# vwxyzjn/cleanrl

Hardware: NVIDIA H100
Metric: env steps/sec (SPS) PPO Breakout num_envs=1024 (higher is better)
Workload: dtype bf16

## Files before the change

### cleanrl_b200/csrc/net_tc.cu

```cuda
#include <cuda.h>
#include <algorithm>
#include "tc_base.cuh"
#include "tc_conv_win.cuh"
#include "tc_conv1_u8.cuh"
#include "tc_gemm_tma.cuh"
#include "tc_wgrad_win.cuh"
#include "tc_reduce.cuh"
#include "tc_aux.cuh"
#include "tc_heads.cuh"
#include "tc_heads_wide.cuh"
#include "tc_lstm.cuh"

namespace b200rl {

struct NatureLayout {
    int A;
    int64_t c1w, c1b, c2w, c2b, c3w, c3b, fcw, fcb, hw, hb, total;
    int64_t w1f, w2f, w2dg, w3f, w3dg, wfcf, wfcdg, w1l, w1sc, packed_total;
    bool wide; int G; int64_t whf, whdg, hbp;
    int64_t wih, whh, bih, bhh, whhp;
    explicit NatureLayout(int A_) : A(A_), wih(-1), whh(-1), bih(-1), bhh(-1), whhp(-1) {
        int64_t o = 0;
        c1w = o; o += 32 * 4 * 8 * 8;  c1b = o; o += 32;
        c2w = o; o += 64 * 32 * 4 * 4; c2b = o; o += 64;
        c3w = o; o += 64 * 64 * 3 * 3; c3b = o; o += 64;
        fcw = o; o += 512 * 3136;      fcb = o; o += 512;
        hw = o;  o += (int64_t)(A + 1) * 512;
        hb = o;  o += A + 1;
        total = o;
        int64_t q = 0;
        w1f = q; q += 32 * 256;
        w2f = q; q += 64 * 512;
        w2dg = q; q += 4 * 32 * 256;
        w3f = q; q += 64 * 576;
        w3dg = q; q += 64 * 576;
        wfcf = q; q += 512 * 3136;
        wfcdg = q; q += 3136 * 512;
        w1l = q; q += 64 * 256 / 2;
        w1sc = q; q += 64 * 2;
        wide = A + 1 > kMaxHeads;
        G = wide ? (int)ceil_div(A + 1, kWideHeadPad) * kWideHeadPad : 0;
        whf = whdg = hbp = 0;
        if (wide) {
            whf = q; q += (int64_t)G * 512;
            whdg = q; q += (int64_t)G * 512;
            hbp = q; q += (int64_t)G * 2;
        }
        packed_total = q;
    }
    struct Lstm {};
    NatureLayout(int A_, Lstm) : A(A_) {
        int64_t o = 0;
        c1w = o; o += 32 * 8 * 8;      c1b = o; o += 32;
        c2w = o; o += 64 * 32 * 4 * 4; c2b = o; o += 64;
        c3w = o; o += 64 * 64 * 3 * 3; c3b = o; o += 64;
        fcw = o; o += 512 * 3136;      fcb = o; o += 512;
        wih = o; o += 512 * 512;       whh = o; o += 512 * 128;
        bih = o; o += 512;             bhh = o; o += 512;
        hw = o;  o += (int64_t)(A + 1) * 128;
        hb = o;  o += A + 1;
        total = o;
        int64_t q = 0;
        w1f = q; q += 32 * 64;
        w2f = q; q += 64 * 512;
        w2dg = q; q += 4 * 32 * 256;
        w3f = q; q += 64 * 576;
        w3dg = q; q += 64 * 576;
        wfcf = q; q += 512 * 3136;
        wfcdg = q; q += 3136 * 512;
        w1l = w1sc = -1;
        wide = true; G = 512;
        whf = q; q += 512 * 512;
        whdg = q; q += 512 * 512;
        hbp = q; q += 512 * 2;
        whhp = q; q += 512 * 128;
        packed_total = q;
    }
};

struct NatureActs {
    int64_t x0, act1, act2, act3, hid, dhid, dact3a, dact3b, dact2a, dact2b, dact1, m1, m2, m3, m4, total;
    explicit NatureActs(int64_t n, bool with_x0 = true) {
        int64_t o = 0;
        x0 = o; if (with_x0) o += n * 28224;
        act1 = o; o += n * 12800;
        act2 = o; o += n * 5184;
        act3 = o; o += n * 3136;
        hid = o;  o += n * 512;
        dhid = o; o += n * 512;
        dact3a = o; o += n * 5184;
        dact3b = o; o += n * 7744;
        dact2a = o; o += n * 6400;
        dact2b = o; o += n * 7744;
        dact1 = o; o += n * 14112;
        auto pad8 = [](int64_t v) { return (v + 7) & ~int64_t(7); };
        m1 = o; o += pad8(n * 100 * 4 * 2);
        m2 = o; o += pad8(n * 81 * 2 * 2);
        m3 = o; o += pad8(n * 49 * 2 * 2);
        m4 = o; o += pad8(n * 16 * 2);
        total = o;
    }
};

static void gemm_rowmajor(KGemmParams& p, const bf16* x, int64_t n, int nchunks) {
    memset(&p, 0, sizeof(p));
    p.scale = 1.f;
    p.A = x; p.M = n; p.nchunks = nchunks;
}


static void win_defaults(WinParams& p) { memset(&p, 0, sizeof(p)); p.scale = 1.f; }
static int round8(int v) { return (v + 7) & ~7; }
static void win_conv1(WinParams& p, const bf16* x0, const int64_t* rows, int64_t n) {
    p.A = x0; p.rows = rows; p.n = (int)n; p.G = 441; p.Wp = 21; p.M = n * 441;
    p.tpi_shift = 2;
    p.n_images = rows ? (int64_t)1 << 24 : n;
    p.ntaps = 4; p.shift[0] = 0; p.shift[1] = 1; p.shift[2] = 21; p.shift[3] = 22; p.WR = round8(128 + 22);
}
static void win_conv2(WinParams& p, const bf16* act1, int64_t n) {
    p.A = act1; p.n = (int)n; p.G = 100; p.Wp = 10; p.M = n * 100;
    p.ntaps = 4; p.shift[0] = 0; p.shift[1] = 1; p.shift[2] = 10; p.shift[3] = 11; p.WR = round8(128 + 11);
}
static void win_conv3(WinParams& p, const bf16* act2, int64_t n) {
    p.A = act2; p.n = (int)n; p.G = 81; p.Wp = 9; p.M = n * 81;
    p.ntaps = 9; for (int ky = 0; ky < 3; ++ky) for (int kx = 0; kx < 3; ++kx) p.shift[ky * 3 + kx] = ky * 9 + kx;
    p.WR = round8(128 + 20);
}
static void wgw_defaults(WGradWinParams& w) { memset(&w, 0, sizeof(w)); }

static const int kC1Ctas = 264, kC2Ctas = 132, kC3Ctas = 132;
static WPlan conv1_wgrad_plan(int64_t n, bool u8) {
    return u8 ? wgrad_plan(n * 512, kC2Ctas, 512) : wgrad_plan(n * 512, kC1Ctas, 128);
}
static WPlan conv2_wgrad_plan(int64_t n) { return wgrad_plan(n * 100, kC2Ctas, 128); }
static WPlan conv3_wgrad_plan(int64_t n) { return wgrad_plan(n * 81, kC3Ctas, 128); }

static size_t wgrad_win_bytes(int splits, int nslots) { return (size_t)splits * nslots * 64 * 64 * sizeof(float); }
static size_t wgrad_win_bias_bytes(int splits) { return (size_t)splits * 64 * sizeof(float); }
static int launch_wgrad_win(const WGradWinParams& p, int ctas, cudaStream_t s, const char* what) {
    const size_t smem = (size_t)kWgradWinStages * ((size_t)p.WRX * 128 * p.cpr + 128 * 128) + 4096 + 1024;
    static SmemAttrCache attr;
    if (int rc0 = attr.ensure(tc_wgrad_win, smem, what)) return rc0;
    CUtensorMap tmX, tmY;
    memset(&tmX, 0, sizeof(tmX)); memset(&tmY, 0, sizeof(tmY));
    const int use_tma = p.tpi_shift ? 0 : 1;
    if (p.rows_per_cta % 128 != 0) return fail(B200RL_ERR_INVALID_ARGUMENT, "%s: rows per CTA must be a multiple of 128", what);
    if (ctas < 1 || (int64_t)(ctas - 1) * p.rows_per_cta >= p.M)
        return fail(B200RL_ERR_INVALID_ARGUMENT, "%s: every row split must own at least one row", what);
    int rc;
    if (use_tma) {
        if (p.rows || p.ldy != 64 || p.ncolsY != 64)
            return fail(B200RL_ERR_INVALID_ARGUMENT, "%s: linear-grid mode needs contiguous rows and 64-channel dY", what);
        if ((rc = make_tmap_2d(&tmX, p.X, p.M, (int64_t)p.cpr * 64, p.WRX, what))) return rc;
        if ((rc = make_tmap_2d(&tmY, p.Y, p.M, 64, 128, what))) return rc;
    } else {
        if ((128 << p.tpi_shift) < p.G) return fail(B200RL_ERR_INVALID_ARGUMENT, "%s: steps per image too small", what);
        if ((rc = make_tmap_3d(&tmX, p.X, p.n_images, p.G, (int64_t)p.cpr * 64, p.WRX, what))) return rc;
    }
    const dim3 grid((unsigned)ceil_div(p.nslots / 2, kWgradWinTilesPerCta), ctas);
    tc_wgrad_win<<<grid, kWgradWinThreads, smem, s>>>(tmX, tmY, p, use_tma);
    return check_launch(what);
}

}

using namespace b200rl;

namespace b200rl {
static bool head_ok(int A) { return A >= 1 && A < kMaxWideHeads; }
static size_t wide_dhead_bytes(int64_t n, const NatureLayout& L) { return ((size_t)n * L.G * 2 + 255) & ~(size_t)255; }
static size_t wide_small_bytes(int64_t n, const NatureLayout& L, int A1) {
    return wide_dhead_bytes(n, L) + colsum_f32_ws(n, A1);
}

static int trunk_fwd(const NatureLayout& L, const NatureActs& Q, const float* params, const bf16* P, bf16* act, int64_t n,
                     cudaStream_t s) {
    int rc;
    KGemmParams p;
    WinParams wp;
    win_defaults(wp); win_conv2(wp, act + Q.act1, n);
    wp.Bw = P + L.w2f; wp.N = 64; wp.vH = 9; wp.vW = 9; wp.out_mode = WOUT_DENSE; wp.out = act + Q.act2;
    wp.bias = params + L.c2b; wp.relu = 1; wp.mask_out = reinterpret_cast<uint32_t*>(act + Q.m2);
    { ProfScope ps(s, "conv2_fwd", 2.0 * n * 81 * 64 * 512, (double)n * ((12800 + 5184) * 2 + 648));
      if ((rc = launch_conv_win_t<128, 2, 2, 4>(wp, s, "naturecnn/conv2"))) return rc; }
    win_defaults(wp); win_conv3(wp, act + Q.act2, n);
    wp.Bw = P + L.w3f; wp.N = 64; wp.vH = 7; wp.vW = 7; wp.out_mode = WOUT_DENSE; wp.out = act + Q.act3;
    wp.bias = params + L.c3b; wp.relu = 1; wp.mask_out = reinterpret_cast<uint32_t*>(act + Q.m3);
    { ProfScope ps(s, "conv3_fwd", 2.0 * n * 49 * 64 * 576, (double)n * ((5184 + 3136) * 2 + 392));
      if ((rc = launch_conv_win_t<128, 1, 4, 9>(wp, s, "naturecnn/conv3"))) return rc; }
    gemm_rowmajor(p, act + Q.act3, n, 49);
    p.Bw = P + L.wfcf; p.N = 512; p.out = act + Q.hid; p.ldo = 512; p.bias = params + L.fcb; p.relu = 1;
    p.mask_out = reinterpret_cast<uint32_t*>(act + Q.m4);
    { ProfScope ps(s, "fc_fwd", 2.0 * n * 512 * 3136, (double)n * (3136 + 512) * 2 + 512.0 * 3136 * 2);
      if (n <= 8192) { if ((rc = launch_gemm_tma<64, 6>(p, s, "naturecnn/fc"))) return rc; }
      else if ((rc = launch_gemm_tma<128, 4>(p, s, "naturecnn/fc"))) return rc; }
    return B200RL_OK;
}

static int trunk_bwd(const NatureLayout& L, const NatureActs& Q, const bf16* P, bf16* act, float* grads, int64_t n,
                     float* wsbig, float* wssmall, void* tail_ready_event, bool dact1_fused, cudaStream_t s) {
    int rc;
    KGemmParams p;
    {
        int splits;
        { ProfScope ps(s, "fc_wgrad", 2.0 * n * 512 * 3136, (double)n * (3136 + 512) * 2 + 512.0 * 3136 * 4);
          if ((splits = launch_wgrad_tma(act + Q.dhid, 512, act + Q.act3, 3136, n, wsbig, s, "naturecnn/fc_wgrad")) < 0) return splits; }
        { ProfScope ps(s, "wgrad_fold_bias", 0, 0);
          note_launches(1); tc_fold_fc<<<(unsigned)ceil_div((int64_t)512 * 3136, 256), 256, 0, s>>>(wsbig, splits, 512, 13 * 256, 512, 3136, 64, 49, 1.f, grads + L.fcw);
          if ((rc = colsum(act + Q.dhid, n, 512, 512, wssmall, grads + L.fcb, s))) return rc; }
        if (tail_ready_event) {
            cudaError_t e = cudaEventRecord(reinterpret_cast<cudaEvent_t>(tail_ready_event), s);
            if (e != cudaSuccess) return fail(B200RL_ERR_CUDA, "naturecnn_backward: cudaEventRecord: %s", cudaGetErrorString(e));
        }
        gemm_rowmajor(p, act + Q.dhid, n, 8);
        p.Bw = P + L.wfcdg; p.N = 3136; p.out = act + Q.dact3a; p.out2 = act + Q.dact3b; p.dual_dact3 = 1;
        p.ldo = 3136; p.mask_bits = reinterpret_cast<const uint32_t*>(act + Q.m3);
        { ProfScope ps(s, "fc_dgrad", 2.0 * n * 512 * 3136, (double)n * ((3136 + 512) * 2 + 392) + 512.0 * 3136 * 2);
          if ((rc = launch_gemm_tma<128, 4>(p, s, "naturecnn/fc_dgrad"))) return rc; }
    }
    WGradWinParams gw;
    WinParams wp;
    FoldWin fw;
    {
        wgw_defaults(gw);
        gw.X = act + Q.act2; gw.M = n * 81; gw.n = (int)n; gw.G = 81; gw.cpr = 1; gw.nslots = 10; gw.WRX = round8(128 + 20);
        for (int t = 0; t < 9; ++t) gw.shift[t] = (t / 3) * 9 + (t % 3);
        const int st[10] = {0, 1, 2, 3, 4, 5, 6, 7, 7, 8};
        for (int k = 0; k < 10; ++k) { gw.slot_tap[k] = st[k]; gw.slot_cc[k] = 0; }
        gw.Y = act + Q.dact3a; gw.ldy = 64; gw.ncolsY = 64;
        const WPlan pl = conv3_wgrad_plan(n);
        gw.rows_per_cta = pl.rows_per_cta; gw.ws = wsbig; gw.wsb = wssmall;
        { ProfScope ps(s, "conv3_wgrad", 2.0 * n * 49 * 64 * 576, (double)n * (5184 + 5184) * 2);
          if ((rc = launch_wgrad_win(gw, pl.splits, s, "naturecnn/conv3_wgrad"))) return rc; }
        memset(&fw, 0, sizeof(fw));
        fw.layer = 3; fw.S = pl.splits; fw.nslots = 10; fw.Cout = 64; fw.scale = 1.f; fw.bscale = 1.f;
        for (int k = 0; k < 10; ++k) { fw.slot_tap[k] = st[k]; fw.slot_skip[k] = (k == 8); }
        { ProfScope ps(s, "wgrad_fold_bias", 0, 0);
          fw.wsb = wssmall; fw.db = grads + L.c3b;
          tc_fold_win<<<(unsigned)ceil_div(640 * 64 + 64, 32), 256, 0, s>>>(wsbig, fw, grads + L.c3w);
          if ((rc = check_launch("naturecnn/conv3_fold"))) return rc; }
        win_defaults(wp);
        wp.A = act + Q.dact3b; wp.n = (int)n; wp.G = 121; wp.Wp = 11; wp.M = n * 121; wp.ntaps = 9;
        for (int ky = 0; ky < 3; ++ky) for (int kx = 0; kx < 3; ++kx) wp.shift[ky * 3 + kx] = (2 - ky) * 11 + (2 - kx);
        wp.WR = round8(128 + 24);
        wp.Bw = P + L.w3dg; wp.N = 64; wp.vH = 9; wp.vW = 9; wp.out_mode = WOUT_DACT2;
        wp.out = act + Q.dact2a; wp.out2 = act + Q.dact2b; wp.mask_bits = reinterpret_cast<const uint32_t*>(act + Q.m2);
        { ProfScope ps(s, "conv3_dgrad", 2.0 * n * 81 * 64 * 576, (double)n * ((7744 + 6400 + 7744) * 2 + 648));
          if ((rc = launch_conv_win_t<128, 1, 4, 9>(wp, s, "naturecnn/conv3_dgrad"))) return rc; }
    }
    {
        wgw_defaults(gw);
        gw.X = act + Q.act1; gw.M = n * 100; gw.n = (int)n; gw.G = 100; gw.cpr = 2; gw.nslots = 8; gw.WRX = round8(128 + 11);
        gw.shift[0] = 0; gw.shift[1] = 1; gw.shift[2] = 10; gw.shift[3] = 11;
        for (int k = 0; k < 8; ++k) { gw.slot_tap[k] = k >> 1; gw.slot_cc[k] = k & 1; }
        gw.Y = act + Q.dact2a; gw.ldy = 64; gw.ncolsY = 64;
        const WPlan pl = conv2_wgrad_plan(n);
        gw.rows_per_cta = pl.rows_per_cta; gw.ws = wsbig; gw.wsb = wssmall;
        { ProfScope ps(s, "conv2_wgrad", 2.0 * n * 81 * 64 * 512, (double)n * (12800 + 6400) * 2);
          if ((rc = launch_wgrad_win(gw, pl.splits, s, "naturecnn/conv2_wgrad"))) return rc; }
        memset(&fw, 0, sizeof(fw));
        fw.layer = 2; fw.S = pl.splits; fw.nslots = 8; fw.Cout = 64; fw.scale = 1.f; fw.bscale = 1.f;
        for (int k = 0; k < 8; ++k) { fw.slot_tap[k] = k >> 1; fw.slot_cc[k] = k & 1; }
        { ProfScope ps(s, "wgrad_fold_bias", 0, 0);
          fw.wsb = wssmall; fw.db = grads + L.c2b;
          tc_fold_win<<<(unsigned)ceil_div(512 * 64 + 64, 32), 256, 0, s>>>(wsbig, fw, grads + L.c2w);
          if ((rc = check_launch("naturecnn/conv2_fold"))) return rc; }
        if (dact1_fused) return B200RL_OK;
        win_defaults(wp);
        wp.A = act + Q.dact2b; wp.n = (int)n; wp.G = 121; wp.Wp = 11; wp.M = n * 121; wp.ntaps = 4;
        for (int a = 0; a < 2; ++a) for (int b = 0; b < 2; ++b) wp.shift[a * 2 + b] = (1 - a) * 11 + (1 - b);
        wp.WR = round8(128 + 12);
        wp.Bw = P + L.w2dg; wp.N = 128; wp.vH = 10; wp.vW = 10; wp.out_mode = WOUT_DACT1;
        wp.out = act + Q.dact1; wp.mask_bits = reinterpret_cast<const uint32_t*>(act + Q.m1);
        { ProfScope ps(s, "conv2_dgrad", 2.0 * n * 400 * 32 * 256, (double)n * ((7744 + 14112) * 2 + 1600));
          if ((rc = launch_conv_win<128, 1, 4, 4>(wp, s, "naturecnn/conv2_dgrad"))) return rc; }
    }
    return B200RL_OK;
}
static size_t trunk_big_bytes(int64_t n) {
    return std::max({wgrad_tma_bytes(n, 512, 3136), wgrad_win_bytes(conv3_wgrad_plan(n).splits, 10),
                     wgrad_win_bytes(conv2_wgrad_plan(n).splits, 8)});
}
static size_t trunk_small_bytes(int64_t n) {
    return std::max({colsum_ws(n, 512), wgrad_win_bias_bytes(conv3_wgrad_plan(n).splits),
                     wgrad_win_bias_bytes(conv2_wgrad_plan(n).splits)});
}

static int wide_head_fwd(const NatureLayout& L, const bf16* P, const bf16* hid, int64_t n, int A1, float* out, cudaStream_t s) {
    KGemmParams p;
    gemm_rowmajor(p, hid, n, 8);
    p.Bw = P + L.whf; p.N = L.G; p.bias = reinterpret_cast<const float*>(P + L.hbp);
    p.out_f32 = out; p.ldo = A1; p.ncols_f32 = A1;
    return launch_gemm_tma<128, 4>(p, s, "wide_heads");
}

static int wide_head_bwd(const NatureLayout& L, const bf16* P, const float* dhead, int64_t n, int A1, const bf16* hid, bf16* dhid,
                         const uint32_t* hid_bits, float* dW, float* db, float* wsbig, float* wssmall, cudaStream_t s) {
    int rc;
    KGemmParams p;
    bf16* dh16 = reinterpret_cast<bf16*>(wssmall);
    float* dbpart = reinterpret_cast<float*>(reinterpret_cast<char*>(wssmall) + wide_dhead_bytes(n, L));
    int cb = (int)ceil_div(n * L.G, 256); if (cb > num_sms() * 8) cb = num_sms() * 8;
    tc_head_dhead_bf16<<<cb, 256, 0, s>>>(dhead, n, A1, L.G, dh16);
    if ((rc = check_launch("wide_heads_dhead"))) return rc;
    if ((rc = colsum_f32(dhead, n, A1, dbpart, db, s))) return rc;
    const int splits = launch_wgrad_tma(dh16, L.G, hid, 512, n, wsbig, s, "wide_heads_wgrad");
    if (splits < 0) return splits;
    tc_fold_fc<<<(unsigned)ceil_div((int64_t)A1 * 512, 256), 256, 0, s>>>(wsbig, splits, L.G, 512, A1, 512, 512, 1, 1.f, dW);
    if ((rc = check_launch("wide_heads_wgrad"))) return rc;
    gemm_rowmajor(p, dh16, n, L.G / 64);
    p.Bw = P + L.whdg; p.N = 512; p.out = dhid; p.ldo = 512;
    p.mask_bits = hid_bits;
    if (n <= 8192) { if ((rc = launch_gemm_tma<64, 6>(p, s, "wide_heads_dgrad"))) return rc; }
// ... 391 lines not shown
```

### cleanrl_b200/csrc/tc_wgmma.cuh

```cuda
#pragma once
#include <cstdint>

namespace b200rl { namespace tc {

__device__ __forceinline__ void wgmma_fence() { asm volatile("wgmma.fence.sync.aligned;" ::: "memory"); }
__device__ __forceinline__ void wgmma_commit() { asm volatile("wgmma.commit_group.sync.aligned;" ::: "memory"); }
template <int N>
__device__ __forceinline__ void wgmma_wait() { asm volatile("wgmma.wait_group.sync.aligned %0;" ::"n"(N) : "memory"); }
template <class T, int R>
__device__ __forceinline__ void wgmma_fence_operands(T (&d)[R]) {
#pragma unroll
    for (int i = 0; i < R; ++i) asm volatile("" : "+r"(reinterpret_cast<uint32_t&>(d[i]))::"memory");
}

template <int N, int TA, int TB> struct WgmmaBf16;
template <int TA, int TB> struct WgmmaBf16<32, TA, TB> {
    __device__ __forceinline__ static void mma(float (&d)[16], uint64_t adesc, uint64_t bdesc, uint32_t accumulate) {
        asm volatile(
            "{\n\t.reg .pred p;\n\tsetp.ne.b32 p, %18, 0;\n\t"
            "wgmma.mma_async.sync.aligned.m64n32k16.f32.bf16.bf16 {"
            "%0, %1, %2, %3, %4, %5, %6, %7, %8, %9, %10, %11, %12, %13, %14, %15"
            "}, %16, %17, p, 1, 1, %19, %20;\n\t}\n"
            : "+f"(d[0]), "+f"(d[1]), "+f"(d[2]), "+f"(d[3]), "+f"(d[4]), "+f"(d[5]), "+f"(d[6]), "+f"(d[7]),
              "+f"(d[8]), "+f"(d[9]), "+f"(d[10]), "+f"(d[11]), "+f"(d[12]), "+f"(d[13]), "+f"(d[14]), "+f"(d[15])
            : "l"(adesc), "l"(bdesc), "r"(accumulate), "n"(TA), "n"(TB));
    }
};
template <int TA, int TB> struct WgmmaBf16<64, TA, TB> {
    __device__ __forceinline__ static void mma(float (&d)[32], uint64_t adesc, uint64_t bdesc, uint32_t accumulate) {
        asm volatile(
            "{\n\t.reg .pred p;\n\tsetp.ne.b32 p, %34, 0;\n\t"
            "wgmma.mma_async.sync.aligned.m64n64k16.f32.bf16.bf16 {"
            "%0, %1, %2, %3, %4, %5, %6, %7, %8, %9, %10, %11, %12, %13, %14, %15, "
            "%16, %17, %18, %19, %20, %21, %22, %23, %24, %25, %26, %27, %28, %29, %30, %31"
            "}, %32, %33, p, 1, 1, %35, %36;\n\t}\n"
            : "+f"(d[0]), "+f"(d[1]), "+f"(d[2]), "+f"(d[3]), "+f"(d[4]), "+f"(d[5]), "+f"(d[6]), "+f"(d[7]),
              "+f"(d[8]), "+f"(d[9]), "+f"(d[10]), "+f"(d[11]), "+f"(d[12]), "+f"(d[13]), "+f"(d[14]), "+f"(d[15]),
              "+f"(d[16]), "+f"(d[17]), "+f"(d[18]), "+f"(d[19]), "+f"(d[20]), "+f"(d[21]), "+f"(d[22]), "+f"(d[23]),
              "+f"(d[24]), "+f"(d[25]), "+f"(d[26]), "+f"(d[27]), "+f"(d[28]), "+f"(d[29]), "+f"(d[30]), "+f"(d[31])
            : "l"(adesc), "l"(bdesc), "r"(accumulate), "n"(TA), "n"(TB));
    }
};
template <int TA, int TB> struct WgmmaBf16<128, TA, TB> {
    __device__ __forceinline__ static void mma(float (&d)[64], uint64_t adesc, uint64_t bdesc, uint32_t accumulate) {
        asm volatile(
            "{\n\t.reg .pred p;\n\tsetp.ne.b32 p, %66, 0;\n\t"
            "wgmma.mma_async.sync.aligned.m64n128k16.f32.bf16.bf16 {"
            "%0, %1, %2, %3, %4, %5, %6, %7, %8, %9, %10, %11, %12, %13, %14, %15, "
            "%16, %17, %18, %19, %20, %21, %22, %23, %24, %25, %26, %27, %28, %29, %30, %31, "
            "%32, %33, %34, %35, %36, %37, %38, %39, %40, %41, %42, %43, %44, %45, %46, %47, "
            "%48, %49, %50, %51, %52, %53, %54, %55, %56, %57, %58, %59, %60, %61, %62, %63"
            "}, %64, %65, p, 1, 1, %67, %68;\n\t}\n"
            : "+f"(d[0]), "+f"(d[1]), "+f"(d[2]), "+f"(d[3]), "+f"(d[4]), "+f"(d[5]), "+f"(d[6]), "+f"(d[7]),
              "+f"(d[8]), "+f"(d[9]), "+f"(d[10]), "+f"(d[11]), "+f"(d[12]), "+f"(d[13]), "+f"(d[14]), "+f"(d[15]),
              "+f"(d[16]), "+f"(d[17]), "+f"(d[18]), "+f"(d[19]), "+f"(d[20]), "+f"(d[21]), "+f"(d[22]), "+f"(d[23]),
              "+f"(d[24]), "+f"(d[25]), "+f"(d[26]), "+f"(d[27]), "+f"(d[28]), "+f"(d[29]), "+f"(d[30]), "+f"(d[31]),
              "+f"(d[32]), "+f"(d[33]), "+f"(d[34]), "+f"(d[35]), "+f"(d[36]), "+f"(d[37]), "+f"(d[38]), "+f"(d[39]),
              "+f"(d[40]), "+f"(d[41]), "+f"(d[42]), "+f"(d[43]), "+f"(d[44]), "+f"(d[45]), "+f"(d[46]), "+f"(d[47]),
              "+f"(d[48]), "+f"(d[49]), "+f"(d[50]), "+f"(d[51]), "+f"(d[52]), "+f"(d[53]), "+f"(d[54]), "+f"(d[55]),
              "+f"(d[56]), "+f"(d[57]), "+f"(d[58]), "+f"(d[59]), "+f"(d[60]), "+f"(d[61]), "+f"(d[62]), "+f"(d[63])
            : "l"(adesc), "l"(bdesc), "r"(accumulate), "n"(TA), "n"(TB));
    }
};
template <int TA, int TB> struct WgmmaBf16<256, TA, TB> {
    __device__ __forceinline__ static void mma(float (&d)[128], uint64_t adesc, uint64_t bdesc, uint32_t accumulate) {
        asm volatile(
            "{\n\t.reg .pred p;\n\tsetp.ne.b32 p, %130, 0;\n\t"
            "wgmma.mma_async.sync.aligned.m64n256k16.f32.bf16.bf16 {"
            "%0, %1, %2, %3, %4, %5, %6, %7, %8, %9, %10, %11, %12, %13, %14, %15, "
            "%16, %17, %18, %19, %20, %21, %22, %23, %24, %25, %26, %27, %28, %29, %30, %31, "
            "%32, %33, %34, %35, %36, %37, %38, %39, %40, %41, %42, %43, %44, %45, %46, %47, "
            "%48, %49, %50, %51, %52, %53, %54, %55, %56, %57, %58, %59, %60, %61, %62, %63, "
            "%64, %65, %66, %67, %68, %69, %70, %71, %72, %73, %74, %75, %76, %77, %78, %79, "
            "%80, %81, %82, %83, %84, %85, %86, %87, %88, %89, %90, %91, %92, %93, %94, %95, "
            "%96, %97, %98, %99, %100, %101, %102, %103, %104, %105, %106, %107, %108, %109, %110, %111, "
            "%112, %113, %114, %115, %116, %117, %118, %119, %120, %121, %122, %123, %124, %125, %126, %127"
            "}, %128, %129, p, 1, 1, %131, %132;\n\t}\n"
            : "+f"(d[0]), "+f"(d[1]), "+f"(d[2]), "+f"(d[3]), "+f"(d[4]), "+f"(d[5]), "+f"(d[6]), "+f"(d[7]),
              "+f"(d[8]), "+f"(d[9]), "+f"(d[10]), "+f"(d[11]), "+f"(d[12]), "+f"(d[13]), "+f"(d[14]), "+f"(d[15]),
              "+f"(d[16]), "+f"(d[17]), "+f"(d[18]), "+f"(d[19]), "+f"(d[20]), "+f"(d[21]), "+f"(d[22]), "+f"(d[23]),
              "+f"(d[24]), "+f"(d[25]), "+f"(d[26]), "+f"(d[27]), "+f"(d[28]), "+f"(d[29]), "+f"(d[30]), "+f"(d[31]),
              "+f"(d[32]), "+f"(d[33]), "+f"(d[34]), "+f"(d[35]), "+f"(d[36]), "+f"(d[37]), "+f"(d[38]), "+f"(d[39]),
              "+f"(d[40]), "+f"(d[41]), "+f"(d[42]), "+f"(d[43]), "+f"(d[44]), "+f"(d[45]), "+f"(d[46]), "+f"(d[47]),
              "+f"(d[48]), "+f"(d[49]), "+f"(d[50]), "+f"(d[51]), "+f"(d[52]), "+f"(d[53]), "+f"(d[54]), "+f"(d[55]),
              "+f"(d[56]), "+f"(d[57]), "+f"(d[58]), "+f"(d[59]), "+f"(d[60]), "+f"(d[61]), "+f"(d[62]), "+f"(d[63]),
              "+f"(d[64]), "+f"(d[65]), "+f"(d[66]), "+f"(d[67]), "+f"(d[68]), "+f"(d[69]), "+f"(d[70]), "+f"(d[71]),
              "+f"(d[72]), "+f"(d[73]), "+f"(d[74]), "+f"(d[75]), "+f"(d[76]), "+f"(d[77]), "+f"(d[78]), "+f"(d[79]),
              "+f"(d[80]), "+f"(d[81]), "+f"(d[82]), "+f"(d[83]), "+f"(d[84]), "+f"(d[85]), "+f"(d[86]), "+f"(d[87]),
              "+f"(d[88]), "+f"(d[89]), "+f"(d[90]), "+f"(d[91]), "+f"(d[92]), "+f"(d[93]), "+f"(d[94]), "+f"(d[95]),
              "+f"(d[96]), "+f"(d[97]), "+f"(d[98]), "+f"(d[99]), "+f"(d[100]), "+f"(d[101]), "+f"(d[102]), "+f"(d[103]),
              "+f"(d[104]), "+f"(d[105]), "+f"(d[106]), "+f"(d[107]), "+f"(d[108]), "+f"(d[109]), "+f"(d[110]), "+f"(d[111]),
              "+f"(d[112]), "+f"(d[113]), "+f"(d[114]), "+f"(d[115]), "+f"(d[116]), "+f"(d[117]), "+f"(d[118]), "+f"(d[119]),
              "+f"(d[120]), "+f"(d[121]), "+f"(d[122]), "+f"(d[123]), "+f"(d[124]), "+f"(d[125]), "+f"(d[126]), "+f"(d[127])
            : "l"(adesc), "l"(bdesc), "r"(accumulate), "n"(TA), "n"(TB));
    }
};

__device__ __forceinline__ void wgmma_u8s8_n64(int (&d)[32], uint64_t adesc, uint64_t bdesc, uint32_t accumulate) {
    asm volatile(
        "{\n\t.reg .pred p;\n\tsetp.ne.b32 p, %34, 0;\n\t"
        "wgmma.mma_async.sync.aligned.m64n64k32.s32.u8.s8 {"
        "%0, %1, %2, %3, %4, %5, %6, %7, %8, %9, %10, %11, %12, %13, %14, %15, "
        "%16, %17, %18, %19, %20, %21, %22, %23, %24, %25, %26, %27, %28, %29, %30, %31"
        "}, %32, %33, p;\n\t}\n"
        : "+r"(d[0]), "+r"(d[1]), "+r"(d[2]), "+r"(d[3]), "+r"(d[4]), "+r"(d[5]), "+r"(d[6]), "+r"(d[7]),
          "+r"(d[8]), "+r"(d[9]), "+r"(d[10]), "+r"(d[11]), "+r"(d[12]), "+r"(d[13]), "+r"(d[14]), "+r"(d[15]),
          "+r"(d[16]), "+r"(d[17]), "+r"(d[18]), "+r"(d[19]), "+r"(d[20]), "+r"(d[21]), "+r"(d[22]), "+r"(d[23]),
          "+r"(d[24]), "+r"(d[25]), "+r"(d[26]), "+r"(d[27]), "+r"(d[28]), "+r"(d[29]), "+r"(d[30]), "+r"(d[31])
        : "l"(adesc), "l"(bdesc), "r"(accumulate));
}

__device__ __forceinline__ void wgmma_f16_rs_n64_tb(float (&d)[32], const uint32_t (&a)[4], uint64_t bdesc, uint32_t accumulate) {
    asm volatile(
        "{\n\t.reg .pred p;\n\tsetp.ne.b32 p, %37, 0;\n\t"
        "wgmma.mma_async.sync.aligned.m64n64k16.f32.f16.f16 {"
        "%0, %1, %2, %3, %4, %5, %6, %7, %8, %9, %10, %11, %12, %13, %14, %15, "
        "%16, %17, %18, %19, %20, %21, %22, %23, %24, %25, %26, %27, %28, %29, %30, %31"
        "}, {%32, %33, %34, %35}, %36, p, 1, 1, 1;\n\t}\n"
        : "+f"(d[0]), "+f"(d[1]), "+f"(d[2]), "+f"(d[3]), "+f"(d[4]), "+f"(d[5]), "+f"(d[6]), "+f"(d[7]),
          "+f"(d[8]), "+f"(d[9]), "+f"(d[10]), "+f"(d[11]), "+f"(d[12]), "+f"(d[13]), "+f"(d[14]), "+f"(d[15]),
          "+f"(d[16]), "+f"(d[17]), "+f"(d[18]), "+f"(d[19]), "+f"(d[20]), "+f"(d[21]), "+f"(d[22]), "+f"(d[23]),
          "+f"(d[24]), "+f"(d[25]), "+f"(d[26]), "+f"(d[27]), "+f"(d[28]), "+f"(d[29]), "+f"(d[30]), "+f"(d[31])
        : "r"(a[0]), "r"(a[1]), "r"(a[2]), "r"(a[3]), "l"(bdesc), "r"(accumulate));
}

}}
```

### cleanrl_b200/csrc/tc_wgrad_win.cuh

```cuda
#pragma once
#include "tc_base.cuh"

namespace b200rl {
using namespace tc;

constexpr int kWgradWinStages = 3;
struct WGradWinParams {
    const bf16* X; const int64_t* rows; int64_t M; int n, G;
    int tpi_shift;
    int64_t n_images;
    int cpr;
    int nslots;
    int slot_tap[16], slot_cc[16];
    int shift[16];
    int WRX;
    const bf16* Y; int ldy, ncolsY;
    int64_t rows_per_cta;
    float* ws;
    float* wsb;
};

constexpr int kWgradWinThreads = 512;
constexpr int kWgradWinTilesPerCta = 2;

template <int NT>
__device__ __forceinline__ void wgrad_win_mma(const WGradWinParams& p, uint8_t* smem, int stage_bytes, int XBYTES, int IMGX,
                                              uint64_t* full_bar, uint64_t* empty_bar, int nsteps, int t0, int w, int tid) {
    constexpr int R = 128, STAGES = kWgradWinStages, NY = 64;
    const int wt = tid & 127;
    uint32_t arel[NT];
#pragma unroll
    for (int tt = 0; tt < NT; ++tt) {
        const int slot = 2 * (t0 + tt) + w;
        arel[tt] = (uint32_t)(p.slot_cc[slot] * IMGX + p.shift[p.slot_tap[slot]] * 128);
    }
    float d[NT][NY / 2];
#pragma unroll
    for (int tt = 0; tt < NT; ++tt)
#pragma unroll
        for (int e = 0; e < NY / 2; ++e) d[tt][e] = 0.f;
    auto step = [&](int it) {
        const int s = it % STAGES;
        mbar_wait(&full_bar[s], (it / STAGES) & 1);
        wgmma_fence();
        const uint32_t xa = smem_u32(smem + (size_t)s * stage_bytes), ya = xa + XBYTES;
        const uint64_t yd = desc_mnmajor(ya, 0);
#pragma unroll
        for (int tt = 0; tt < NT; ++tt) {
            const uint64_t xd = desc_mnmajor(xa + arel[tt], 0);
#pragma unroll
            for (int kk = 0; kk < R / 16; ++kk)
                WgmmaBf16<NY, 1, 1>::mma(d[tt], xd + kk * 128, yd + kk * 128, (it | kk) != 0 ? 1u : 0u);
        }
        wgmma_commit();
    };
    for (int it = 0; it + 1 < nsteps; ++it) {
        step(it);
        wgmma_wait<1>();
        if (it > 0 && (tid & 31) == 0) mbar_arrive(&empty_bar[(it - 1) % STAGES]);
    }
    step(nsteps - 1);
    wgmma_wait<0>();
    const int row = ((wt >> 5) << 4) + ((wt & 31) >> 2), col = (wt & 3) * 2;
    float* wsb = p.ws + (int64_t)blockIdx.y * (p.nslots * 64) * NY;
#pragma unroll
    for (int tt = 0; tt < NT; ++tt) {
        wgmma_fence_operands(d[tt]);
        float* d0 = wsb + (int64_t)((2 * (t0 + tt) + w) * 64 + row) * NY + col;
#pragma unroll
        for (int j = 0; j < NY / 8; ++j) {
            *reinterpret_cast<float2*>(d0 + 8 * j) = make_float2(d[tt][4 * j], d[tt][4 * j + 1]);
            *reinterpret_cast<float2*>(d0 + 8 * NY + 8 * j) = make_float2(d[tt][4 * j + 2], d[tt][4 * j + 3]);
        }
    }
}

static __global__ void __launch_bounds__(kWgradWinThreads, 1) tc_wgrad_win(const __grid_constant__ CUtensorMap tmX, const __grid_constant__ CUtensorMap tmY,
                                                       const WGradWinParams p, int use_tma) {
    constexpr int R = 128, STAGES = kWgradWinStages, LOOKAHEAD = 1, NY = 64, TT = kWgradWinTilesPerCta;
    static_assert(TT == 2, "the wgmma warpgroups dispatch on 1 or 2 tiles per CTA");
    extern __shared__ uint8_t smem_raw[];
    __shared__ uint64_t full_bar[STAGES], empty_bar[STAGES];
    uint8_t* smem = reinterpret_cast<uint8_t*>((reinterpret_cast<uintptr_t>(smem_raw) + 1023) & ~uintptr_t(1023));
    const int tid = threadIdx.x, warp = tid >> 5;
    const int IMGX = p.WRX * 128;
    const int XBYTES = IMGX * p.cpr;
    const int stage_bytes = XBYTES + R * 128;
    const int xt = p.nslots / 2;
    const int t0 = blockIdx.x * TT;
    float* sRed = reinterpret_cast<float*>(smem + (size_t)STAGES * stage_bytes);
    if (tid == 0) {
        for (int s = 0; s < STAGES; ++s) { mbar_init(&full_bar[s], use_tma ? 1 : 5); mbar_init(&empty_bar[s], (use_tma ? 4 : 0) + 8); }
        fence_barrier_init();
        tma_prefetch_desc(&tmX);
        if (use_tma) tma_prefetch_desc(&tmY);
    }
    __syncthreads();
    const int64_t m_begin = (int64_t)blockIdx.y * p.rows_per_cta;
    int64_t m_end = m_begin + p.rows_per_cta;
    if (m_end > p.M) m_end = p.M;
    const int nsteps = m_end > m_begin ? (int)((m_end - m_begin + R - 1) / R) : 0;
    const int tmask = (1 << p.tpi_shift) - 1;
    const int64_t g0 = m_begin / R;

    if (warp == 4) {
        if ((tid & 31) == 0) {
            int z_next = 0;
            if (!use_tma && nsteps > 0) {
                const int64_t img = g0 >> p.tpi_shift;
                z_next = p.rows ? (int)__ldg(p.rows + (img < p.n ? img : 0)) : (int)img;
            }
            for (int it = 0; it < nsteps; ++it) {
                const int s = it % STAGES;
                const int z = z_next;
                if (!use_tma && it + 1 < nsteps) {
                    const int64_t img1 = (g0 + it + 1) >> p.tpi_shift;
                    z_next = p.rows ? (int)__ldg(p.rows + (img1 < p.n ? img1 : 0)) : (int)img1;
                }
                if (it >= STAGES) mbar_wait(&empty_bar[s], ((it / STAGES) - 1) & 1);
                const uint32_t dst = smem_u32(smem + (size_t)s * stage_bytes);
                if (use_tma) {
                    const int m0 = (int)(m_begin + (int64_t)it * R);
                    mbar_arrive_expect_tx(&full_bar[s], (uint32_t)stage_bytes);
                    for (int c = 0; c < p.cpr; ++c) tma_load_2d(dst + c * IMGX, &tmX, c * 64, m0, &full_bar[s]);
                    tma_load_2d(dst + XBYTES, &tmY, 0, m0, &full_bar[s]);
                } else {
                    const int t_in = (int)((g0 + it) & tmask);
                    mbar_arrive_expect_tx(&full_bar[s], (uint32_t)XBYTES);
                    for (int c = 0; c < p.cpr; ++c) tma_load_3d(dst + c * IMGX, &tmX, c * 64, t_in * 128, z, &full_bar[s]);
                }
            }
        }
    } else if (warp < 4) {
        const int rq = tid >> 3, c16 = tid & 7;
        float bsum[8];
#pragma unroll
        for (int e = 0; e < 8; ++e) bsum[e] = 0.f;
        auto add_step = [&](const uint8_t* sYp) {
#pragma unroll
            for (int ps = 0; ps < R / 16; ++ps) {
                const int rr = ps * 16 + rq;
                const int4 v = *reinterpret_cast<const int4*>(sYp + img_off(rr, c16));
                const uint32_t w[4] = {(uint32_t)v.x, (uint32_t)v.y, (uint32_t)v.z, (uint32_t)v.w};
#pragma unroll
                for (int e = 0; e < 4; ++e) {
                    bsum[2 * e] += __uint_as_float(w[e] << 16);
                    bsum[2 * e + 1] += __uint_as_float(w[e] & 0xFFFF0000u);
                }
            }
        };
        if (use_tma) {
            for (int it = 0; it < nsteps; ++it) {
                const int s = it % STAGES;
                mbar_wait(&full_bar[s], (it / STAGES) & 1);
                add_step(smem + (size_t)s * stage_bytes + XBYTES);
                __syncwarp();
                if ((tid & 31) == 0) mbar_arrive(&empty_bar[s]);
            }
        } else {
            for (int it = 0; it < nsteps; ++it) {
                const int s = it % STAGES;
                const int64_t g = g0 + it;
                const int64_t img = g >> p.tpi_shift;
                const int t_in = (int)(g & tmask);
                if (it >= STAGES) mbar_wait(&empty_bar[s], ((it / STAGES) - 1) & 1);
                const uint32_t sY = smem_u32(smem + (size_t)s * stage_bytes + XBYTES);
#pragma unroll
                for (int ps = 0; ps < R / 16; ++ps) {
                    const int rr = ps * 16 + rq;
                    const int rl = t_in * 128 + rr;
                    const int col = c16 * 8;
                    const bool ok = rl < p.G && img < p.n && col < p.ncolsY;
                    cp_async16(sY + img_off(rr, c16), p.Y + (ok ? (img * p.G + rl) * (int64_t)p.ldy + col : 0), ok ? 16u : 0u);
                }
                cp_async_commit();
                if (it >= LOOKAHEAD) {
                    cp_async_wait<LOOKAHEAD>();
                    const int sd = (it - LOOKAHEAD) % STAGES;
                    add_step(smem + (size_t)sd * stage_bytes + XBYTES);
                    fence_proxy_async_smem();
                    __syncwarp();
                    if ((tid & 31) == 0) mbar_arrive(&full_bar[sd]);
                }
            }
            cp_async_wait<0>();
            for (int d = (nsteps >= LOOKAHEAD ? nsteps - LOOKAHEAD : 0); d < nsteps; ++d)
                add_step(smem + (size_t)(d % STAGES) * stage_bytes + XBYTES);
            fence_proxy_async_smem();
            __syncwarp();
            if ((tid & 31) == 0)
                for (int d = (nsteps >= LOOKAHEAD ? nsteps - LOOKAHEAD : 0); d < nsteps; ++d) mbar_arrive(&full_bar[d % STAGES]);
        }
#pragma unroll
        for (int e = 0; e < 8; ++e) sRed[rq * 64 + c16 * 8 + e] = bsum[e];
        asm volatile("bar.sync 1, 128;" ::: "memory");
        if (tid < 64) {
            float t = 0.f;
#pragma unroll
            for (int l = 0; l < 16; ++l) t += sRed[l * 64 + tid];
            if (blockIdx.x == 0) p.wsb[(int64_t)blockIdx.y * NY + tid] = t;
        }
    } else if (warp >= 8) {
        const int w = (warp - 8) >> 2;
        if (xt - t0 >= TT) wgrad_win_mma<TT>(p, smem, stage_bytes, XBYTES, IMGX, full_bar, empty_bar, nsteps, t0, w, tid);
        else wgrad_win_mma<1>(p, smem, stage_bytes, XBYTES, IMGX, full_bar, empty_bar, nsteps, t0, w, tid);
    }
}

}
```

Before: 1.197 million.

## Add templated linear-grid wgrad kernel computing a whole kernel row per wgmma

Splits the windowed weight-gradient kernel into the existing 3D-TMA per-image path and a new templated linear-grid kernel for conv2/conv3. In the new kernel each warpgroup covers a full kernel row of consecutive taps with one wide wgmma (N=64*taps, adding an m64n192 instruction), so each staged X/dY tile is reused across taps. The kernel uses one 2D grid axis, a dedicated bias-reduction pair of warps and a deeper stage count. Register pressure rises from 96-float accumulators per channel chunk, and unsupported tap/chunk combinations now fail instead of falling back.

```diff
diff --git a/cleanrl_b200/csrc/net_tc.cu b/cleanrl_b200/csrc/net_tc.cu
--- a/cleanrl_b200/csrc/net_tc.cu
+++ b/cleanrl_b200/csrc/net_tc.cu
@@ -137,28 +137,44 @@
 
 static size_t wgrad_win_bytes(int splits, int nslots) { return (size_t)splits * nslots * 64 * 64 * sizeof(float); }
 static size_t wgrad_win_bias_bytes(int splits) { return (size_t)splits * 64 * sizeof(float); }
+template <int TPR, int CPR, int NWG, int STAGES>
+static int launch_wgrad_win_t(const WGradWinParams& p, const CUtensorMap& tmX, const CUtensorMap& tmY, int ctas, cudaStream_t s,
+                              const char* what) {
+    for (int t = 0; t < TPR * NWG; ++t)
+        if (p.shift[t] != p.shift[t - t % TPR] + t % TPR)
+            return fail(B200RL_ERR_INVALID_ARGUMENT, "%s: the taps of a kernel row must be consecutive grid rows", what);
+    const size_t smem = (size_t)STAGES * ((size_t)p.WRX * 128 * CPR + 128 * 128) + 4096 + 1024;
+    static SmemAttrCache attr;
+    if (int rc = attr.ensure(tc_wgrad_win_t<TPR, CPR, NWG, STAGES>, smem, what)) return rc;
+    tc_wgrad_win_t<TPR, CPR, NWG, STAGES><<<ctas, 128 * (1 + NWG), smem, s>>>(tmX, tmY, p);
+    return check_launch(what);
+}
 static int launch_wgrad_win(const WGradWinParams& p, int ctas, cudaStream_t s, const char* what) {
-    const size_t smem = (size_t)kWgradWinStages * ((size_t)p.WRX * 128 * p.cpr + 128 * 128) + 4096 + 1024;
-    static SmemAttrCache attr;
-    if (int rc0 = attr.ensure(tc_wgrad_win, smem, what)) return rc0;
     CUtensorMap tmX, tmY;
     memset(&tmX, 0, sizeof(tmX)); memset(&tmY, 0, sizeof(tmY));
-    const int use_tma = p.tpi_shift ? 0 : 1;
     if (p.rows_per_cta % 128 != 0) return fail(B200RL_ERR_INVALID_ARGUMENT, "%s: rows per CTA must be a multiple of 128", what);
     if (ctas < 1 || (int64_t)(ctas - 1) * p.rows_per_cta >= p.M)
         return fail(B200RL_ERR_INVALID_ARGUMENT, "%s: every row split must own at least one row", what);
     int rc;
-    if (use_tma) {
+    if (!p.tpi_shift) {
         if (p.rows || p.ldy != 64 || p.ncolsY != 64)
             return fail(B200RL_ERR_INVALID_ARGUMENT, "%s: linear-grid mode needs contiguous rows and 64-channel dY", what);
         if ((rc = make_tmap_2d(&tmX, p.X, p.M, (int64_t)p.cpr * 64, p.WRX, what))) return rc;
         if ((rc = make_tmap_2d(&tmY, p.Y, p.M, 64, 128, what))) return rc;
-    } else {
-        if ((128 << p.tpi_shift) < p.G) return fail(B200RL_ERR_INVALID_ARGUMENT, "%s: steps per image too small", what);
-        if ((rc = make_tmap_3d(&tmX, p.X, p.n_images, p.G, (int64_t)p.cpr * 64, p.WRX, what))) return rc;
-    }
+        int ntaps = 0;
+        for (int k = 0; k < p.nslots; ++k) ntaps = std::max(ntaps, p.slot_tap[k] + 1);
+        if (p.cpr == 1 && ntaps == 9) return launch_wgrad_win_t<3, 1, 3, 5>(p, tmX, tmY, ctas, s, what);
+        if (p.cpr == 2 && ntaps == 4) return launch_wgrad_win_t<2, 2, 2, 4>(p, tmX, tmY, ctas, s, what);
+        return fail(B200RL_ERR_INVALID_ARGUMENT, "%s: no linear-grid weight-gradient kernel for %d taps x %d channel chunks", what,
+                    ntaps, p.cpr);
+    }
+    if ((128 << p.tpi_shift) < p.G) return fail(B200RL_ERR_INVALID_ARGUMENT, "%s: steps per image too small", what);
+    if ((rc = make_tmap_3d(&tmX, p.X, p.n_images, p.G, (int64_t)p.cpr * 64, p.WRX, what))) return rc;
+    const size_t smem = (size_t)kWgradWinStages * ((size_t)p.WRX * 128 * p.cpr + 128 * 128) + 4096 + 1024;
+    static SmemAttrCache attr;
+    if ((rc = attr.ensure(tc_wgrad_win, smem, what))) return rc;
     const dim3 grid((unsigned)ceil_div(p.nslots / 2, kWgradWinTilesPerCta), ctas);
-    tc_wgrad_win<<<grid, kWgradWinThreads, smem, s>>>(tmX, tmY, p, use_tma);
+    tc_wgrad_win<<<grid, kWgradWinThreads, smem, s>>>(tmX, p);
     return check_launch(what);
 }
 
diff --git a/cleanrl_b200/csrc/tc_wgmma.cuh b/cleanrl_b200/csrc/tc_wgmma.cuh
--- a/cleanrl_b200/csrc/tc_wgmma.cuh
+++ b/cleanrl_b200/csrc/tc_wgmma.cuh
@@ -59,6 +59,33 @@
               "+f"(d[40]), "+f"(d[41]), "+f"(d[42]), "+f"(d[43]), "+f"(d[44]), "+f"(d[45]), "+f"(d[46]), "+f"(d[47]),
               "+f"(d[48]), "+f"(d[49]), "+f"(d[50]), "+f"(d[51]), "+f"(d[52]), "+f"(d[53]), "+f"(d[54]), "+f"(d[55]),
               "+f"(d[56]), "+f"(d[57]), "+f"(d[58]), "+f"(d[59]), "+f"(d[60]), "+f"(d[61]), "+f"(d[62]), "+f"(d[63])
+            : "l"(adesc), "l"(bdesc), "r"(accumulate), "n"(TA), "n"(TB));
+    }
+};
+template <int TA, int TB> struct WgmmaBf16<192, TA, TB> {
+    __device__ __forceinline__ static void mma(float (&d)[96], uint64_t adesc, uint64_t bdesc, uint32_t accumulate) {
+        asm volatile(
+            "{\n\t.reg .pred p;\n\tsetp.ne.b32 p, %98, 0;\n\t"
+            "wgmma.mma_async.sync.aligned.m64n192k16.f32.bf16.bf16 {"
+            "%0, %1, %2, %3, %4, %5, %6, %7, %8, %9, %10, %11, %12, %13, %14, %15, "
+            "%16, %17, %18, %19, %20, %21, %22, %23, %24, %25, %26, %27, %28, %29, %30, %31, "
+            "%32, %33, %34, %35, %36, %37, %38, %39, %40, %41, %42, %43, %44, %45, %46, %47, "
+            "%48, %49, %50, %51, %52, %53, %54, %55, %56, %57, %58, %59, %60, %61, %62, %63, "
+            "%64, %65, %66, %67, %68, %69, %70, %71, %72, %73, %74, %75, %76, %77, %78, %79, "
+            "%80, %81, %82, %83, %84, %85, %86, %87, %88, %89, %90, %91, %92, %93, %94, %95"
+            "}, %96, %97, p, 1, 1, %99, %100;\n\t}\n"
+            : "+f"(d[0]), "+f"(d[1]), "+f"(d[2]), "+f"(d[3]), "+f"(d[4]), "+f"(d[5]), "+f"(d[6]), "+f"(d[7]),
+              "+f"(d[8]), "+f"(d[9]), "+f"(d[10]), "+f"(d[11]), "+f"(d[12]), "+f"(d[13]), "+f"(d[14]), "+f"(d[15]),
+              "+f"(d[16]), "+f"(d[17]), "+f"(d[18]), "+f"(d[19]), "+f"(d[20]), "+f"(d[21]), "+f"(d[22]), "+f"(d[23]),
+              "+f"(d[24]), "+f"(d[25]), "+f"(d[26]), "+f"(d[27]), "+f"(d[28]), "+f"(d[29]), "+f"(d[30]), "+f"(d[31]),
+              "+f"(d[32]), "+f"(d[33]), "+f"(d[34]), "+f"(d[35]), "+f"(d[36]), "+f"(d[37]), "+f"(d[38]), "+f"(d[39]),
+              "+f"(d[40]), "+f"(d[41]), "+f"(d[42]), "+f"(d[43]), "+f"(d[44]), "+f"(d[45]), "+f"(d[46]), "+f"(d[47]),
+              "+f"(d[48]), "+f"(d[49]), "+f"(d[50]), "+f"(d[51]), "+f"(d[52]), "+f"(d[53]), "+f"(d[54]), "+f"(d[55]),
+              "+f"(d[56]), "+f"(d[57]), "+f"(d[58]), "+f"(d[59]), "+f"(d[60]), "+f"(d[61]), "+f"(d[62]), "+f"(d[63]),
+              "+f"(d[64]), "+f"(d[65]), "+f"(d[66]), "+f"(d[67]), "+f"(d[68]), "+f"(d[69]), "+f"(d[70]), "+f"(d[71]),
+              "+f"(d[72]), "+f"(d[73]), "+f"(d[74]), "+f"(d[75]), "+f"(d[76]), "+f"(d[77]), "+f"(d[78]), "+f"(d[79]),
+              "+f"(d[80]), "+f"(d[81]), "+f"(d[82]), "+f"(d[83]), "+f"(d[84]), "+f"(d[85]), "+f"(d[86]), "+f"(d[87]),
+              "+f"(d[88]), "+f"(d[89]), "+f"(d[90]), "+f"(d[91]), "+f"(d[92]), "+f"(d[93]), "+f"(d[94]), "+f"(d[95])
             : "l"(adesc), "l"(bdesc), "r"(accumulate), "n"(TA), "n"(TB));
     }
 };
diff --git a/cleanrl_b200/csrc/tc_wgrad_win.cuh b/cleanrl_b200/csrc/tc_wgrad_win.cuh
--- a/cleanrl_b200/csrc/tc_wgrad_win.cuh
+++ b/cleanrl_b200/csrc/tc_wgrad_win.cuh
@@ -75,8 +75,7 @@
     }
 }
 
-static __global__ void __launch_bounds__(kWgradWinThreads, 1) tc_wgrad_win(const __grid_constant__ CUtensorMap tmX, const __grid_constant__ CUtensorMap tmY,
-                                                       const WGradWinParams p, int use_tma) {
+static __global__ void __launch_bounds__(kWgradWinThreads, 1) tc_wgrad_win(const __grid_constant__ CUtensorMap tmX, const WGradWinParams p) {
     constexpr int R = 128, STAGES = kWgradWinStages, LOOKAHEAD = 1, NY = 64, TT = kWgradWinTilesPerCta;
     static_assert(TT == 2, "the wgmma warpgroups dispatch on 1 or 2 tiles per CTA");
     extern __shared__ uint8_t smem_raw[];
@@ -90,10 +89,9 @@
     const int t0 = blockIdx.x * TT;
     float* sRed = reinterpret_cast<float*>(smem + (size_t)STAGES * stage_bytes);
     if (tid == 0) {
-        for (int s = 0; s < STAGES; ++s) { mbar_init(&full_bar[s], use_tma ? 1 : 5); mbar_init(&empty_bar[s], (use_tma ? 4 : 0) + 8); }
+        for (int s = 0; s < STAGES; ++s) { mbar_init(&full_bar[s], 5); mbar_init(&empty_bar[s], 8); }
         fence_barrier_init();
         tma_prefetch_desc(&tmX);
-        if (use_tma) tma_prefetch_desc(&tmY);
     }
     __syncthreads();
     const int64_t m_begin = (int64_t)blockIdx.y * p.rows_per_cta;
@@ -106,29 +104,22 @@
     if (warp == 4) {
         if ((tid & 31) == 0) {
             int z_next = 0;
-            if (!use_tma && nsteps > 0) {
+            if (nsteps > 0) {
                 const int64_t img = g0 >> p.tpi_shift;
                 z_next = p.rows ? (int)__ldg(p.rows + (img < p.n ? img : 0)) : (int)img;
             }
             for (int it = 0; it < nsteps; ++it) {
                 const int s = it % STAGES;
                 const int z = z_next;
-                if (!use_tma && it + 1 < nsteps) {
+                if (it + 1 < nsteps) {
                     const int64_t img1 = (g0 + it + 1) >> p.tpi_shift;
                     z_next = p.rows ? (int)__ldg(p.rows + (img1 < p.n ? img1 : 0)) : (int)img1;
                 }
                 if (it >= STAGES) mbar_wait(&empty_bar[s], ((it / STAGES) - 1) & 1);
                 const uint32_t dst = smem_u32(smem + (size_t)s * stage_bytes);
-                if (use_tma) {
-                    const int m0 = (int)(m_begin + (int64_t)it * R);
-                    mbar_arrive_expect_tx(&full_bar[s], (uint32_t)stage_bytes);
-                    for (int c = 0; c < p.cpr; ++c) tma_load_2d(dst + c * IMGX, &tmX, c * 64, m0, &full_bar[s]);
-                    tma_load_2d(dst + XBYTES, &tmY, 0, m0, &full_bar[s]);
-                } else {
-                    const int t_in = (int)((g0 + it) & tmask);
-                    mbar_arrive_expect_tx(&full_bar[s], (uint32_t)XBYTES);
-                    for (int c = 0; c < p.cpr; ++c) tma_load_3d(dst + c * IMGX, &tmX, c * 64, t_in * 128, z, &full_bar[s]);
-                }
+                const int t_in = (int)((g0 + it) & tmask);
+                mbar_arrive_expect_tx(&full_bar[s], (uint32_t)XBYTES);
+                for (int c = 0; c < p.cpr; ++c) tma_load_3d(dst + c * IMGX, &tmX, c * 64, t_in * 128, z, &full_bar[s]);
             }
         }
     } else if (warp < 4) {
@@ -149,48 +140,38 @@
                 }
             }
         };
-        if (use_tma) {
-            for (int it = 0; it < nsteps; ++it) {
-                const int s = it % STAGES;
-                mbar_wait(&full_bar[s], (it / STAGES) & 1);
-                add_step(smem + (size_t)s * stage_bytes + XBYTES);
+        for (int it = 0; it < nsteps; ++it) {
+            const int s = it % STAGES;
+            const int64_t g = g0 + it;
+            const int64_t img = g >> p.tpi_shift;
+            const int t_in = (int)(g & tmask);
+            if (it >= STAGES) mbar_wait(&empty_bar[s], ((it / STAGES) - 1) & 1);
+            const uint32_t sY = smem_u32(smem + (size_t)s * stage_bytes + XBYTES);
+#pragma unroll
+            for (int ps = 0; ps < R / 16; ++ps) {
+                const int rr = ps * 16 + rq;
+                const int rl = t_in * 128 + rr;
+                const int col = c16 * 8;
+                const bool ok = rl < p.G && img < p.n && col < p.ncolsY;
+                cp_async16(sY + img_off(rr, c16), p.Y + (ok ? (img * p.G + rl) * (int64_t)p.ldy + col : 0), ok ? 16u : 0u);
+            }
+            cp_async_commit();
+            if (it >= LOOKAHEAD) {
+                cp_async_wait<LOOKAHEAD>();
+                const int sd = (it - LOOKAHEAD) % STAGES;
+                add_step(smem + (size_t)sd * stage_bytes + XBYTES);
+                fence_proxy_async_smem();
                 __syncwarp();
-                if ((tid & 31) == 0) mbar_arrive(&empty_bar[s]);
-            }
-        } else {
-            for (int it = 0; it < nsteps; ++it) {
-                const int s = it % STAGES;
-                const int64_t g = g0 + it;
-                const int64_t img = g >> p.tpi_shift;
-                const int t_in = (int)(g & tmask);
-                if (it >= STAGES) mbar_wait(&empty_bar[s], ((it / STAGES) - 1) & 1);
-                const uint32_t sY = smem_u32(smem + (size_t)s * stage_bytes + XBYTES);
-#pragma unroll
-                for (int ps = 0; ps < R / 16; ++ps) {
-                    const int rr = ps * 16 + rq;
-                    const int rl = t_in * 128 + rr;
-                    const int col = c16 * 8;
-                    const bool ok = rl < p.G && img < p.n && col < p.ncolsY;
-                    cp_async16(sY + img_off(rr, c16), p.Y + (ok ? (img * p.G + rl) * (int64_t)p.ldy + col : 0), ok ? 16u : 0u);
-                }
-                cp_async_commit();
-                if (it >= LOOKAHEAD) {
-                    cp_async_wait<LOOKAHEAD>();
-                    const int sd = (it - LOOKAHEAD) % STAGES;
-                    add_step(smem + (size_t)sd * stage_bytes + XBYTES);
-                    fence_proxy_async_smem();
-                    __syncwarp();
-                    if ((tid & 31) == 0) mbar_arrive(&full_bar[sd]);
-                }
-            }
-            cp_async_wait<0>();
-            for (int d = (nsteps >= LOOKAHEAD ? nsteps - LOOKAHEAD : 0); d < nsteps; ++d)
-                add_step(smem + (size_t)(d % STAGES) * stage_bytes + XBYTES);
-            fence_proxy_async_smem();
-            __syncwarp();
-            if ((tid & 31) == 0)
-                for (int d = (nsteps >= LOOKAHEAD ? nsteps - LOOKAHEAD : 0); d < nsteps; ++d) mbar_arrive(&full_bar[d % STAGES]);
-        }
+                if ((tid & 31) == 0) mbar_arrive(&full_bar[sd]);
+            }
+        }
+        cp_async_wait<0>();
+        for (int d = (nsteps >= LOOKAHEAD ? nsteps - LOOKAHEAD : 0); d < nsteps; ++d)
+            add_step(smem + (size_t)(d % STAGES) * stage_bytes + XBYTES);
+        fence_proxy_async_smem();
+        __syncwarp();
+        if ((tid & 31) == 0)
+            for (int d = (nsteps >= LOOKAHEAD ? nsteps - LOOKAHEAD : 0); d < nsteps; ++d) mbar_arrive(&full_bar[d % STAGES]);
 #pragma unroll
         for (int e = 0; e < 8; ++e) sRed[rq * 64 + c16 * 8 + e] = bsum[e];
         asm volatile("bar.sync 1, 128;" ::: "memory");
@@ -207,4 +188,131 @@
     }
 }
 
+template <int TPR, int CPR, int NWG, int STAGES>
+static __global__ void __launch_bounds__(128 * (1 + NWG), 1)
+tc_wgrad_win_t(const __grid_constant__ CUtensorMap tmX, const __grid_constant__ CUtensorMap tmY, const WGradWinParams p) {
+    constexpr int R = 128, NY = 64, N = 64 * TPR;
+    extern __shared__ uint8_t smem_raw[];
+    __shared__ uint64_t full_bar[STAGES], empty_bar[STAGES];
+    uint8_t* smem = reinterpret_cast<uint8_t*>((reinterpret_cast<uintptr_t>(smem_raw) + 1023) & ~uintptr_t(1023));
+    const int tid = threadIdx.x, warp = tid >> 5;
+    const int IMGX = p.WRX * 128;
+    const int XBYTES = IMGX * CPR;
+    const int stage_bytes = XBYTES + R * 128;
+    float* sRed = reinterpret_cast<float*>(smem + (size_t)STAGES * stage_bytes);
+    if (tid == 0) {
+        for (int s = 0; s < STAGES; ++s) { mbar_init(&full_bar[s], 1); mbar_init(&empty_bar[s], 2 + 4 * NWG); }
+        fence_barrier_init();
+        tma_prefetch_desc(&tmX);
+        tma_prefetch_desc(&tmY);
+    }
+    __syncthreads();
+    const int64_t m_begin = (int64_t)blockIdx.x * p.rows_per_cta;
+    int64_t m_end = m_begin + p.rows_per_cta;
+    if (m_end > p.M) m_end = p.M;
+    const int nsteps = (int)((m_end - m_begin + R - 1) / R);
+
+    if (warp == 0) {
+        if (tid == 0) {
+            for (int it = 0; it < nsteps; ++it) {
+                const int s = it % STAGES;
+                if (it >= STAGES) mbar_wait(&empty_bar[s], ((it / STAGES) - 1) & 1);
+                const uint32_t dst = smem_u32(smem + (size_t)s * stage_bytes);
+                const int m0 = (int)(m_begin + (int64_t)it * R);
+                mbar_arrive_expect_tx(&full_bar[s], (uint32_t)stage_bytes);
+#pragma unroll
+                for (int c = 0; c < CPR; ++c) tma_load_2d(dst + c * IMGX, &tmX, c * 64, m0, &full_bar[s]);
+                tma_load_2d(dst + XBYTES, &tmY, 0, m0, &full_bar[s]);
+            }
+        }
+    } else if (warp < 3) {
+        const int bt = tid - 32, rq = bt >> 3, c16 = bt & 7;
+        float bsum[2][8];
+#pragma unroll
+        for (int h = 0; h < 2; ++h)
+#pragma unroll
+            for (int e = 0; e < 8; ++e) bsum[h][e] = 0.f;
+        for (int it = 0; it < nsteps; ++it) {
+            const int s = it % STAGES;
+            mbar_wait(&full_bar[s], (it / STAGES) & 1);
+            const uint8_t* sYp = smem + (size_t)s * stage_bytes + XBYTES;
+#pragma unroll
+            for (int ps = 0; ps < R / 16; ++ps)
+#pragma unroll
+                for (int h = 0; h < 2; ++h) {
+                    const int4 v = *reinterpret_cast<const int4*>(sYp + img_off(ps * 16 + 8 * h + rq, c16));
+                    const uint32_t w[4] = {(uint32_t)v.x, (uint32_t)v.y, (uint32_t)v.z, (uint32_t)v.w};
+#pragma unroll
+                    for (int e = 0; e < 4; ++e) {
+                        bsum[h][2 * e] += __uint_as_float(w[e] << 16);
+                        bsum[h][2 * e + 1] += __uint_as_float(w[e] & 0xFFFF0000u);
+                    }
+                }
+            __syncwarp();
+            if ((tid & 31) == 0) mbar_arrive(&empty_bar[s]);
+        }
+#pragma unroll
+        for (int h = 0; h < 2; ++h)
+#pragma unroll
+            for (int e = 0; e < 8; ++e) sRed[(8 * h + rq) * 64 + c16 * 8 + e] = bsum[h][e];
+        named_bar(1, 64);
+        float t = 0.f;
+#pragma unroll
+        for (int l = 0; l < 16; ++l) t += sRed[l * 64 + bt];
+        p.wsb[(int64_t)blockIdx.x * NY + bt] = t;
+    } else if (warp >= 4) {
+        const int w = (warp - 4) >> 2, wt = tid & 127;
+        const uint32_t xrow = (uint32_t)p.shift[w * TPR] * 128;
+        float d[CPR][N / 2];
+#pragma unroll
+        for (int c = 0; c < CPR; ++c)
+#pragma unroll
+            for (int e = 0; e < N / 2; ++e) d[c][e] = 0.f;
+        auto step = [&](int it) {
+            const int s = it % STAGES;
+            mbar_wait(&full_bar[s], (it / STAGES) & 1);
+            wgmma_fence();
+            const uint32_t xa = smem_u32(smem + (size_t)s * stage_bytes), ya = xa + XBYTES;
+            const uint64_t yd = desc_mnmajor(ya, 0);
+#pragma unroll
+            for (int c = 0; c < CPR; ++c) {
+                const uint64_t xd = desc_mnmajor(xa + c * IMGX + xrow, 128);
+#pragma unroll
+                for (int kk = 0; kk < R / 16; ++kk)
+                    WgmmaBf16<N, 1, 1>::mma(d[c], yd + kk * 128, xd + kk * 128, (it | kk) != 0 ? 1u : 0u);
+            }
+            wgmma_commit();
+        };
+        for (int it = 0; it + 1 < nsteps; ++it) {
+            step(it);
+            wgmma_wait<1>();
+            if (it > 0 && (tid & 31) == 0) mbar_arrive(&empty_bar[(it - 1) % STAGES]);
+        }
+        step(nsteps - 1);
+        wgmma_wait<0>();
+        const int co = ((wt >> 5) << 4) + ((wt & 31) >> 2), ch = (wt & 3) * 2;
+        float* wsp = p.ws + (int64_t)blockIdx.x * (p.nslots * 64) * NY;
+#pragma unroll
+        for (int c = 0; c < CPR; ++c) {
+            wgmma_fence_operands(d[c]);
+#pragma unroll
+            for (int kx = 0; kx < TPR; ++kx) {
+                int slot = -1;
+                for (int s = p.nslots - 1; s >= 0; --s)
+                    if (p.slot_tap[s] == w * TPR + kx && p.slot_cc[s] == c) slot = s;
+                if (slot < 0) continue;
+                float* d0 = wsp + (int64_t)(slot * 64 + ch) * NY + co;
+#pragma unroll
+                for (int j = 0; j < 8; ++j) {
+                    const float* f = &d[c][4 * (8 * kx + j)];
+                    d0[(8 * j) * NY] = f[0];
+                    d0[(8 * j + 1) * NY] = f[1];
+                    d0[(8 * j) * NY + 8] = f[2];
+                    d0[(8 * j + 1) * NY + 8] = f[3];
+                }
+            }
+        }
+    }
 }
+
+}
```

New measurement: 1.228 million, median of 6. 1.03x the previous value.
